# PositronicsLab/Moby

Measured on NVIDIA B200. Metric: env_steps_per_s, higher is better.
Workload: dtype f64

## Files before the change

include/b200moby.h:

```cpp
#ifndef B200MOBY_H
#define B200MOBY_H

#ifdef __cplusplus
extern "C" {
#endif

#define B200MOBY_ABI_VERSION 3

typedef enum {
  B200MOBY_OK = 0,
  B200MOBY_ERR_INVALID = 1,
  B200MOBY_ERR_CUDA = 2,
  B200MOBY_ERR_UNSUPPORTED = 3,
  B200MOBY_ERR_NO_DEVICE = 4
} b200moby_status;

enum {
  B200MOBY_LCP_OK = 0,
  B200MOBY_LCP_TRIVIAL = 1,
  B200MOBY_LCP_RAY = 2,
  B200MOBY_LCP_MAXITER = 3,
  B200MOBY_LCP_SINGULAR = 4,
  B200MOBY_LCP_EMPTY_RATIO = 5,
  B200MOBY_LCP_UNVERIFIED = 6,
// ... 100 lines not shown
b200moby_status b200moby_get_time(b200moby_handle h, double* t);
b200moby_status b200moby_get_last_lcp(b200moby_handle h, int* n, double* z, int zcap);

#define B200MOBY_MAX_KERNELS 20
typedef struct {
  char name[48];
  double ms;
  long long launches;
  long long envs;
  long long flops;
  long long lcp_solves;
  int lcp_nmax;
  int threads_per_env;
} b200moby_kernel_stat;
typedef struct {
  int n_kernels;
  b200moby_kernel_stat k[B200MOBY_MAX_KERNELS];
} b200moby_kernel_profile;
b200moby_status b200moby_get_kernel_profile(b200moby_handle h, int enable, int reset, b200moby_kernel_profile* out);

b200moby_status b200moby_get_impact_profile(b200moby_handle h, long long* prof);

b200moby_status b200moby_get_env_stats(b200moby_handle h, int* stat);

b200moby_status b200moby_lcp_lemke_batched(int batch, int n, const double* M_dev, const double* q_dev, double* z_dev,
                                           double piv_tol, double zero_tol, int* status_dev, int* pivots_dev,
                                           int* pivot_log_dev, int log_cap, void* stream);
b200moby_status b200moby_lcp_fast_batched(int batch, int n, const double* M_dev, const double* q_dev, double* z_dev,
                                          int warm_start, double zero_tol, int* status_dev, int* pivots_dev,
                                          int* pivot_log_dev, int log_cap, void* stream);
b200moby_status b200moby_lcp_lemke_regularized_batched(int batch, int n, const double* M_dev, const double* q_dev,
                                                       double* z_dev, int min_exp, int step_exp, int max_exp,
                                                       double piv_tol, double zero_tol, int* status_dev,
                                                       int* pivots_dev, void* stream);
b200moby_status b200moby_lcp_fast_regularized_batched(int batch, int n, const double* M_dev, const double* q_dev,
                                                      double* z_dev, int warm_start, int min_exp, int step_exp,
                                                      int max_exp, double zero_tol, int* status_dev, int* pivots_dev,
                                                      void* stream);
b200moby_status b200moby_lcp_lemke_host(int batch, int n, const double* M, const double* q, double* z, double piv_tol,
                                        double zero_tol, int* status, int* pivots, int device);
b200moby_status b200moby_lcp_fast_host(int batch, int n, const double* M, const double* q, double* z, int warm_start,
                                       double zero_tol, int* status, int* pivots, int device);

b200moby_status b200moby_selftest_div(int n, const double* x_dev, const double* y_dev, double* q_dev, double* qref_dev, void* stream);

b200moby_status b200moby_lcp_solve_host(int mode, int batch, int n, const double* M, const double* q, double* z, int warm_start,
// ... 20 lines not shown
```

moby_b200/capi.py:

```python
import ctypes as C
import os

_HERE = os.path.dirname(os.path.abspath(__file__))
LIB_PATH = os.environ.get("B200MOBY_LIB", os.path.join(_HERE, "libb200moby.so"))


class B200MobyError(RuntimeError):
    pass


class RcDesc(C.Structure):
    _fields_ = [
        ("n_links", C.c_int), ("first_body", C.c_int),
        ("parent", C.POINTER(C.c_int)), ("joint_type", C.POINTER(C.c_int)),
        ("joint_axis", C.POINTER(C.c_double)), ("loc_parent", C.POINTER(C.c_double)), ("loc_child", C.POINTER(C.c_double)),
        ("rel_quat", C.POINTER(C.c_double)),
        ("fdyn_algorithm", C.c_int),
        ("ctrl_kp", C.POINTER(C.c_double)), ("ctrl_kv", C.POINTER(C.c_double)), ("ctrl_amp", C.POINTER(C.c_double)),
        ("ctrl_freq", C.POINTER(C.c_double)),
    ]


class SceneDesc(C.Structure):
    _fields_ = [
# ... 14 lines not shown
    _fields_ = [("name", C.c_char * 48), ("ms", C.c_double), ("launches", C.c_longlong), ("envs", C.c_longlong),
                ("flops", C.c_longlong), ("lcp_solves", C.c_longlong), ("lcp_nmax", C.c_int), ("threads_per_env", C.c_int)]


class KernelProfile(C.Structure):
    _fields_ = [("n_kernels", C.c_int), ("k", KernelStat * 20)]


class Counters(C.Structure):
    _fields_ = [(k, C.c_longlong) for k in (
        "env_steps", "mini_steps", "lcp_solves", "lcp_fast_calls", "lemke_calls", "pivots", "lcp_failures",
        "impact_tol_events", "contacts", "max_lcp_n", "pivot_flops", "ca_iterations", "assembly_flops", "stab_iterations",
        "stab_lcp_solves", "stab_line_search_failures")]

    def as_dict(self):
        return {k: int(getattr(self, k)) for k, _ in self._fields_}


SYMBOLS = [
    "b200moby_last_error", "b200moby_abi_version", "b200moby_device_count",
    "b200moby_create", "b200moby_destroy", "b200moby_set_state", "b200moby_get_state",
    "b200moby_set_state_dev", "b200moby_get_state_dev", "b200moby_step", "b200moby_set_pivot_budget", "b200moby_get_counters",
    "b200moby_reset_counters", "b200moby_get_launch_count", "b200moby_get_time", "b200moby_get_last_lcp",
    "b200moby_get_impact_profile", "b200moby_get_kernel_profile", "b200moby_get_env_stats",
    "b200moby_lcp_lemke_batched", "b200moby_lcp_fast_batched", "b200moby_lcp_lemke_regularized_batched",
    "b200moby_lcp_fast_regularized_batched", "b200moby_lcp_lemke_host", "b200moby_lcp_fast_host", "b200moby_lcp_solve_host",
    "b200moby_selftest_div",
    "b200moby_fwd_dyn_batched", "b200moby_find_contacts_batched", "b200moby_find_contacts_host", "b200moby_delassus_batched",
    "b200moby_set_joint_state", "b200moby_get_joint_state", "b200moby_set_joint_state_dev", "b200moby_get_joint_state_dev",
    "b200moby_set_joint_forces", "b200moby_rc_fwd_dyn_batched", "b200moby_rc_inertia_batched",
]

_lib = None


def lib():
    global _lib
    if _lib is not None:
        return _lib
    if not os.path.exists(LIB_PATH):
        raise B200MobyError(f"{LIB_PATH} not built; run `python -c 'import __graft_entry__ as g; g.build()'` "
                            "(there is no CPU fallback for the hot path)")
    L = C.CDLL(LIB_PATH)
    L.b200moby_last_error.restype = C.c_char_p
    vp, ip, dp = C.c_void_p, C.c_void_p, C.c_void_p
    L.b200moby_create.argtypes = [C.POINTER(SceneDesc), C.c_int, C.POINTER(C.c_void_p)]
    L.b200moby_destroy.argtypes = [C.c_void_p]
    L.b200moby_set_state.argtypes = [C.c_void_p, dp, dp]
    L.b200moby_get_state.argtypes = [C.c_void_p, dp, dp]
    L.b200moby_set_state_dev.argtypes = [C.c_void_p, dp, dp, vp]
    L.b200moby_get_state_dev.argtypes = [C.c_void_p, dp, dp, vp]
    L.b200moby_step.argtypes = [C.c_void_p, C.c_double, C.c_int, vp]
    L.b200moby_set_pivot_budget.argtypes = [C.c_void_p, C.c_int]
    L.b200moby_get_counters.argtypes = [C.c_void_p, C.POINTER(Counters)]
    L.b200moby_reset_counters.argtypes = [C.c_void_p]
    L.b200moby_get_launch_count.argtypes = [C.c_void_p, C.POINTER(C.c_longlong)]
    L.b200moby_get_time.argtypes = [C.c_void_p, dp]
    L.b200moby_get_last_lcp.argtypes = [C.c_void_p, ip, dp, C.c_int]
    L.b200moby_get_impact_profile.argtypes = [C.c_void_p, ip]
    L.b200moby_get_env_stats.argtypes = [C.c_void_p, ip]
    L.b200moby_get_kernel_profile.argtypes = [C.c_void_p, C.c_int, C.c_int, C.POINTER(KernelProfile)]
    L.b200moby_lcp_lemke_batched.argtypes = [C.c_int, C.c_int, dp, dp, dp, C.c_double, C.c_double, ip, ip, ip, C.c_int, vp]
    L.b200moby_lcp_fast_batched.argtypes = [C.c_int, C.c_int, dp, dp, dp, C.c_int, C.c_double, ip, ip, ip, C.c_int, vp]
    L.b200moby_lcp_lemke_regularized_batched.argtypes = [C.c_int, C.c_int, dp, dp, dp, C.c_int, C.c_int, C.c_int,
                                                         C.c_double, C.c_double, ip, ip, vp]
    L.b200moby_lcp_fast_regularized_batched.argtypes = [C.c_int, C.c_int, dp, dp, dp, C.c_int, C.c_int, C.c_int, C.c_int,
                                                        C.c_double, ip, ip, vp]
    L.b200moby_lcp_lemke_host.argtypes = [C.c_int, C.c_int, dp, dp, dp, C.c_double, C.c_double, ip, ip, C.c_int]
    L.b200moby_lcp_fast_host.argtypes = [C.c_int, C.c_int, dp, dp, dp, C.c_int, C.c_double, ip, ip, C.c_int]
    L.b200moby_lcp_solve_host.argtypes = [C.c_int, C.c_int, C.c_int, dp, dp, dp, C.c_int, C.c_double, C.c_double, C.c_int, C.c_int,
                                          C.c_int, ip, ip, C.c_int]
    L.b200moby_selftest_div.argtypes = [C.c_int, dp, dp, dp, dp, vp]
    L.b200moby_fwd_dyn_batched.argtypes = [C.c_void_p, dp, dp, C.c_double, vp]
    L.b200moby_find_contacts_batched.argtypes = [C.c_void_p, dp, dp, C.c_int, ip, dp, dp, dp, dp, ip, dp, vp]
    L.b200moby_find_contacts_host.argtypes = [C.c_void_p, C.c_int, ip, dp, dp, dp, dp, ip, dp]
    L.b200moby_delassus_batched.argtypes = [C.c_void_p, dp, dp, C.c_int, dp, dp, ip, vp]
    L.b200moby_set_joint_state.argtypes = [C.c_void_p, dp, dp]
    L.b200moby_get_joint_state.argtypes = [C.c_void_p, dp, dp]
    L.b200moby_set_joint_state_dev.argtypes = [C.c_void_p, dp, dp, vp]
    L.b200moby_get_joint_state_dev.argtypes = [C.c_void_p, dp, dp, vp]
    L.b200moby_set_joint_forces.argtypes = [C.c_void_p, dp]
    L.b200moby_rc_fwd_dyn_batched.argtypes = [C.c_void_p, C.c_int, dp, dp, dp, dp, vp]
    L.b200moby_rc_inertia_batched.argtypes = [C.c_void_p, dp, dp, vp]
# ... 8 lines not shown
```

moby_b200/csrc/lcp_device.cuh:

```cuda
#pragma once
#include "common.cuh"

namespace b2m {

enum {
  LCP_OK = 0, LCP_TRIVIAL = 1, LCP_RAY = 2, LCP_MAXITER = 3, LCP_SINGULAR = 4, LCP_EMPTY_RATIO = 5,
  LCP_UNVERIFIED = 6, LCP_DEFER = 7, LCP_REGULARIZED = 16
};

B2M_DEV B2M_INL double m_at(const double* M, int ldm, int r, int c, double lambda) {
  double v = M[(size_t)c * ldm + r];
  return (r == c) ? v + lambda : v;
}

template <class G>
B2M_DEV B2M_NOINL double norm_inf(const G& g, int n, const double* M, int ldm, double lambda) {
  double m = 0.0;
  if constexpr (G::size == 1) {
    double m1 = 0.0, m2 = 0.0, m3 = 0.0;
    for (int c = 0; c < n; c++) {
      const double* Mc = M + (size_t)c * ldm;
      int r = 0;
      for (; r + 8 <= n; r += 8) {
        double v0 = Mc[r], v1 = Mc[r + 1], v2 = Mc[r + 2], v3 = Mc[r + 3], v4 = Mc[r + 4], v5 = Mc[r + 5], v6 = Mc[r + 6], v7 = Mc[r + 7];
// ... 664 lines not shown
    }
#endif
    for (int i = j + 1 + g.tid; i < k; i += G::size) {
      const double l = A[(size_t)j * k + i] * rinv;
      A[(size_t)j * k + i] = l;
      for (int c = j + 1; c < k; c++) A[(size_t)c * k + i] = fma(-l, A[(size_t)c * k + j], A[(size_t)c * k + i]);
      b[i] = fma(-l, bj, b[i]);
    }
    g.sync();
  }
  for (int c = k - 1; c >= 0; c--) {
    const double xc = b[c] / A[(size_t)c * k + c];
    g.sync();
    if (g.tid == 0) b[c] = xc;
    for (int i = g.tid; i < c; i += G::size) b[i] = fma(-A[(size_t)c * k + i], xc, b[i]);
    g.sync();
  }
  return true;
}

B2M_DEV inline void list_erase(int* L, int& m, int pos) { for (int i = pos; i + 1 < m; i++) L[i] = L[i + 1]; m--; }
B2M_DEV inline void list_insert_sorted(int* L, int& m, int v) { int i = m; while (i > 0 && L[i - 1] > v) { L[i] = L[i - 1]; i--; } L[i] = v; m++; }

template <class G>
B2M_DEV B2M_NOINL int lcp_fast_solve(const G& g, int n, const double* M, int ldm, const double* q, double lambda, double zero_tol,
                              bool warm, double* z, double* wd, int* wi, int* pivots_out, int* log, int log_cap,
                              int* log_len, int* budget = nullptr, int* executed_out = nullptr, double offdiag = -1.0) {
  double* A = wd;
  double* zz = A + (size_t)n * n;
  double* w = zz + n;
  int* nonbas = wi;
  int* bas = wi + n;
  int* cnt = wi + 2 * n;
  const int W32 = (n + 31) >> 5;
  unsigned* cur = (unsigned*)(wi + 2 * n + 2);
  unsigned* hist = cur + W32;
  int nlog = 0, nh = 0, executed = 0;
  if (executed_out) *executed_out = 0;
  if (zero_tol < 0.0) zero_tol = n * norm_inf_with(g, n, M, ldm, lambda, offdiag) * B2M_EPS;
  if (warm) {
    if (g.tid == 0) {
      int k = 0, nb = 0;
      for (int i = 0; i < W32; i++) cur[i] = 0u;
      for (int i = 0; i < n; i++) { if (fabs(z[i]) < zero_tol) bas[nb++] = i; else { nonbas[k++] = i; cur[i >> 5] |= 1u << (i & 31); } }
      cnt[0] = k; cnt[1] = nb;
    }
  } else {
    double key = B2M_INF; int idx = 0x7fffffff;
    for (int i = g.tid; i < n; i += G::size) { const double x = q[i]; if (x < key) { key = x; idx = i; } }
    g.min_key_idx(key, idx);
    if (key > -zero_tol) {
      for (int i = g.tid; i < n; i += G::size) z[i] = 0.0;
      if (pivots_out) *pivots_out = 0; if (log_len) *log_len = 0;
      g.sync();
      return LCP_TRIVIAL;
    }
    if (g.tid == 0) {
      nonbas[0] = idx; int nb = 0; for (int i = 0; i < n; i++) if (i != idx) bas[nb++] = i; cnt[0] = 1; cnt[1] = nb;
      for (int i = 0; i < W32; i++) cur[i] = 0u;
      cur[idx >> 5] |= 1u << (idx & 31);
    }
  }
  g.sync();
  const int MAX_PIV = 2 * n;
  int piv = 0, status = LCP_MAXITER;
  for (piv = 0; piv < MAX_PIV; piv++) {
    if (budget && --(*budget) < 0) { status = LCP_DEFER; break; }
    {
      bool rep = false;
      if (!log) {
        const int stored = nh < B2M_FAST_HIST ? nh : B2M_FAST_HIST;
        for (int t = g.tid; t < stored; t += G::size) {
          bool eq = true;
          for (int i = 0; i < W32; i++) eq = eq && (hist[t * W32 + i] == cur[i]);
          rep = rep || eq;
        }
      }
      if (g.any(rep)) { piv = MAX_PIV; break; }
      if (!log) { for (int i = g.tid; i < W32; i += G::size) hist[(nh % B2M_FAST_HIST) * W32 + i] = cur[i]; nh++; }
    }
    executed++;
    const int k = cnt[0], nb = cnt[1];
    if (G::size == 32 && k <= 64) {
      const double* __restrict__ Mr = M; const int* __restrict__ nbp = nonbas; double* __restrict__ Ar = A;
      for (int r = g.tid; r < k; r += G::size) {
        const int nr = nbp[r];
#pragma unroll 4
        for (int c = 0; c < k; c++) Ar[c * k + r] = m_at(Mr, ldm, nr, nbp[c], lambda);
      }
    } else if (G::size == 1) {
// ... 171 lines not shown
    case 9: return 1e9;
    case 10: return 1e10;
    case 11: return 1e11;
    case 12: return 1e12;
    case 13: return 1e13;
    case 14: return 1e14;
    case 15: return 1e15;
    case 16: return 1e16;
    case 17: return 1e17;
    case 18: return 1e18;
    case 19: return 1e19;
    case 20: return 1e20;
    case 21: return 1e21;
    case 22: return 1e22;
    case 23: return 1e23;
    case 24: return 1e24;
    default: return pow(10.0, (double)e);
  }
}

template <class G>
B2M_DEV int lcp_fast_regularized(const G& g, int n, const double* M, int ldm, const double* q, double zero_tol, bool warm,
                                    int min_exp, int step_exp, int max_exp, double* z, double* wd, int* wi,
                                    int* pivots_out, long long* stats, int* budget = nullptr) {
  if (n == 0) { if (pivots_out) *pivots_out = 0; return LCP_OK; }
  const double offdiag = norm_inf_offdiag(g, n, M, ldm);
  const double ZERO_TOL = (zero_tol > 0.0) ? zero_tol : n * norm_inf_with(g, n, M, ldm, 0.0, offdiag) * B2M_NEAR_ZERO;
  double* wv = wd + (size_t)n * n + n;
  int total = 0, piv = 0, ex = 0;
  int st = lcp_fast_solve(g, n, M, ldm, q, 0.0, zero_tol, warm, z, wd, wi, &piv, nullptr, 0, nullptr, budget, &ex, offdiag);
  if (st == LCP_DEFER) return st;
  bool zvalid = warm || st == LCP_OK || st == LCP_TRIVIAL;
  total += piv;
  if (stats && g.tid == 0) { stats[0]++; stats[1] += piv; stats[2] += ex; }
  if ((st == LCP_OK || st == LCP_TRIVIAL) && lcp_verify(g, n, M, ldm, q, 0.0, z, ZERO_TOL, false, wv)) {
    if (pivots_out) *pivots_out = piv;
    return st;
  }
  int attempt = 0;
  for (int rf = min_exp; rf < max_exp; rf += step_exp, attempt++) {
    const double lambda = pow10i(rf);
    g.sync();
    st = lcp_fast_solve(g, n, M, ldm, q, lambda, zero_tol, zvalid, z, wd, wi, &piv, nullptr, 0, nullptr, budget, &ex, offdiag);
    if (st == LCP_DEFER) return st;
    zvalid = zvalid || st == LCP_OK || st == LCP_TRIVIAL;
    total += piv;
    if (stats && g.tid == 0) { stats[0]++; stats[1] += piv; stats[2] += ex; }
    if ((st == LCP_OK || st == LCP_TRIVIAL) && lcp_verify(g, n, M, ldm, q, lambda, z, ZERO_TOL, true, wv)) {
      if (pivots_out) *pivots_out = total;
      return LCP_REGULARIZED + attempt;
    }
  }
  if (pivots_out) *pivots_out = total;
  return LCP_UNVERIFIED;
}

template <class G>
B2M_DEV int lcp_lemke_regularized(const G& g, int n, const double* M, int ldm, const double* q, double piv_tol,
                                     double zero_tol, int min_exp, int step_exp, int max_exp, double* z, double* wd,
                                     int* wi, int* pivots_out, long long* stats, int* budget = nullptr) {
  if (n == 0) { if (pivots_out) *pivots_out = 0; return LCP_OK; }
  const double offdiag = norm_inf_offdiag(g, n, M, ldm);
  const double ZERO_TOL = (zero_tol > 0.0) ? zero_tol : n * norm_inf_with(g, n, M, ldm, 0.0, offdiag) * B2M_NEAR_ZERO;
  double* wv = wd + (size_t)n * (n + 2);
  int total = 0, piv = 0, ex = 0;
  int st = lemke_solve(g, n, M, ldm, q, 0.0, piv_tol, zero_tol, z, wd, wi, &piv, nullptr, 0, nullptr, budget, &ex, offdiag);
  if (st == LCP_DEFER) return st;
// ... 210 lines not shown
```

moby_b200/csrc/sim_device.cuh:

```cuda
#pragma once
#include "lcp_device.cuh"
#include "rc_device.cuh"

namespace b2m {

enum { SH_NONE = 0, SH_SPHERE = 1, SH_BOX = 2, SH_PLANE = 3,
       SH_WHEEL = 4,
       SH_PIN = 5, SH_PINWORLD = 6 };
enum { CNT_ENV_STEPS = 0, CNT_MINI_STEPS, CNT_LCP_SOLVES, CNT_FAST_CALLS, CNT_LEMKE_CALLS, CNT_PIVOTS, CNT_LCP_FAIL,
       CNT_IMPACT_TOL, CNT_CONTACTS, CNT_MAX_N, CNT_OVERFLOW, CNT_PIVOT_FLOPS, CNT_ASM_FLOPS, CNT_CA_ITERS, CNT_STAB_ITERS, CNT_STAB_SOLVES, CNT_STAB_LSFAIL, CNT_COUNT };
#define B2M_NKMAX 64
#define B2M_WHEEL_NS_MAX 16
#define B2M_WTAB_OFF ((size_t)4 * (B2M_NKMAX + 1) * (B2M_NKMAX / 2))
#define B2M_MAX_CLASSES 12
#define B2M_SLOT_CONT B2M_MAX_CLASSES
#define B2M_SLOT_STRAGGLER (B2M_MAX_CLASSES + 1)
#define B2M_SLOT_HARD (B2M_MAX_CLASSES + 2)
#define B2M_SLOT_HARD_BACK (B2M_MAX_CLASSES + 3)
#define B2M_SLOTS (B2M_MAX_CLASSES + 4)
#define B2M_ROUNDS_MAX 8
#define B2M_MAX_STALL 64
#ifndef B2M_LEAN
#define B2M_LEAN 0
#endif
// ... 28 lines not shown
  int stab_max_iterations; double stab_eps;
  const double* min_step_env;
  double* q; double* v; double* time; double* zlast; int* zlast_n;
  double* vlast; int* vlast_n;
  unsigned long long* counters;
  int* cost; int hard_cost; int cost_shift;
  int thread_lanes;
  int pivot_budget;
  double* hacc;
  double* hpend;
  int* queue;
  int* qctl;
  int n_classes; int class_nmax[B2M_MAX_CLASSES]; int class_cmax[B2M_MAX_CLASSES];
  int class_budget[B2M_MAX_CLASSES];
  double* tap_MM; double* tap_qq; double* tap_z; int* tap_n;
  const RCTree* rc; int rc_links, rc_first;
  int ngc;
  double* jq; double* jqd; const double* jtau;
  double* gscratch; size_t gstride;
  unsigned long long* kstat; int kslot;
  int* env_stat;
  int tap_times;
  long long* tap_prof;
};

struct EnvMem {
  double *bx, *bq, *bR, *bvl, *bva, *bmass, *bdims, *bJ, *xsave, *qsave;
  double *pd_dist, *pd_pa, *pd_pb;
  double *cp, *cnrm, *ct1, *ct2, *cdist, *cmu, *cmuv, *ceps, *ccomp;
  double *Jr, *XJ, *Xb, *D, *Cv, *imp, *acc, *dv;
  double *MM, *qq, *z, *zl, *vl, *work;
  double *Lf, *gv;
  double *jq, *jqd, *jqsave, *jtau, *rS, *rV;
  int *bshape, *ben, *pair_a, *pair_b, *cb1, *cb2, *cNK, *icon, *cisl, *corder, *isl_start, *gcoff, *bisl, *frow_c, *frow_j, *scal, *iwork;
  int *ranc, *gcb, *gcl;
  long long* prof; long long prof_stride;
  const double* wtab;
  long long dbg[4];
  double cdt;
};

enum { PH_LOAD = 0, PH_CONTACTS, PH_ISLANDS, PH_PROBLEM, PH_BUILD, PH_FAST, PH_LEMKE, PH_APPLY, PH_STORE, PH_COUNT };
#ifdef __CUDA_ARCH__
#define B2M_PROF_T0(m) const long long _pt0 = (m).prof ? clock64() : 0
#define B2M_PROF_ADD(m, g, k) do { if ((m).prof && (g).tid == 0) (m).prof[(k) * (m).prof_stride] += clock64() - _pt0; } while (0)
#else
// ... 38 lines not shown
  m.Jr = nullptr; m.zl = nullptr; m.vl = nullptr; m.prof = nullptr; m.prof_stride = 0; m.gcb = m.gcl = nullptr; m.cdt = 0.0; m.wtab = nullptr;
}
B2M_HD inline void env_carve_impact(EnvMem& m, double* d, int* i, const EnvDims& D) {
  const int nb = D.nb, cmax = D.cmax, nmax = D.nmax;
  if (D.ngc) { m.Jr = d; d += (size_t)3 * cmax * D.ngc; m.XJ = d; d += (size_t)3 * cmax * D.ngc; m.Xb = d; d += (size_t)D.ngc * D.ngc; m.dv = d; d += D.ngc; m.Lf = d; d += (size_t)D.ngc * D.ngc + D.ngc; m.gv = d; d += D.ngc; }
  else { m.Lf = m.gv = nullptr; m.Jr = d; d += 36 * cmax; m.XJ = d; d += 36 * cmax; m.Xb = d; d += 36 * nb; m.dv = d; d += 6 * nb; }
  m.D = d; d += 6 * (size_t)cmax * cmax;
  m.Cv = d; d += 3 * cmax; m.imp = d; d += 3 * cmax; m.acc = d; d += 3 * cmax;
  m.MM = d; d += (size_t)nmax * nmax; m.qq = d; d += nmax; m.z = d; d += nmax; m.zl = d; d += nmax; m.vl = d; d += cmax; m.work = d;
  m.gcoff = i; i += nb; m.bisl = i; i += nb;
  m.icon = i; i += cmax; m.cisl = i; i += cmax; m.corder = i; i += cmax;
  m.isl_start = i; i += nb + 1;
  m.frow_c = i; i += nmax; m.frow_j = i; i += nmax;
  m.gcb = i; i += D.ngc; m.gcl = i; i += D.ngc;
  m.iwork = i;
}
B2M_HD inline void env_carve(EnvMem& m, double* d, int* i, const EnvDims& D) {
  env_carve_small(m, d, i, D);
  env_carve_impact(m, d + env_small_doubles(D), i + env_small_ints(D), D);
}

enum { S_NPAIRS = 0, S_NCON = 1, S_NC = 2, S_NGC = 3, S_N = 4, S_NISL = 5, S_FLAG = 6, S_TMP = 7, S_ZLN = 8, S_ZLDIRTY = 9, S_NTOT = 10, S_VLN = 11, S_VLDIRTY = 12, S_FAILED = 13, S_EXEC = 14 };

struct EnvCtx { int budget; bool limit; void* ladder = nullptr; };

struct EnvStatBase { unsigned long long fail, lemke, fast, solves, pivots; };
B2M_HD B2M_INL EnvStatBase env_stat_base(const unsigned long long* lc);

B2M_HD B2M_INL EnvStatBase env_stat_base(const unsigned long long* lc) {
  EnvStatBase b; b.fail = lc[CNT_LCP_FAIL] + lc[CNT_OVERFLOW]; b.lemke = lc[CNT_LEMKE_CALLS]; b.fast = lc[CNT_FAST_CALLS]; b.solves = lc[CNT_LCP_SOLVES]; b.pivots = lc[CNT_PIVOTS]; return b;
}
template <class G>
B2M_DEV B2M_INL void env_stat_commit(const G& g, const SimParams& P, int e, const unsigned long long* lc, const EnvStatBase& b) {
  if (!P.env_stat || g.tid != 0) return;
  const size_t ne = P.n_envs;
  P.env_stat[e] += (int)(lc[CNT_LCP_FAIL] + lc[CNT_OVERFLOW] - b.fail);
  P.env_stat[ne + e] += (int)(lc[CNT_LEMKE_CALLS] - b.lemke);
  P.env_stat[2 * ne + e] += (int)(lc[CNT_FAST_CALLS] - b.fast);
  P.env_stat[3 * ne + e] += (int)(lc[CNT_LCP_SOLVES] - b.solves);
  P.env_stat[4 * ne + e] += (int)(lc[CNT_PIVOTS] - b.pivots);
}

B2M_HD B2M_INL void quat_to_R(const double* qt, double* R) {
  const double x = qt[0], y = qt[1], z = qt[2], w = qt[3];
  R[0] = 1.0 - 2.0 * (y * y + z * z); R[1] = 2.0 * (x * y - w * z);       R[2] = 2.0 * (x * z + w * y);
  R[3] = 2.0 * (x * y + w * z);       R[4] = 1.0 - 2.0 * (x * x + z * z); R[5] = 2.0 * (y * z - w * x);
  R[6] = 2.0 * (x * z - w * y);       R[7] = 2.0 * (y * z + w * x);       R[8] = 1.0 - 2.0 * (x * x + y * y);
// ... 1146 lines not shown
}

template <class G>
B2M_DEV double min_constraint_velocity(const G& g, const EnvMem& m) {
  const int nc = m.scal[S_NC];
  double v = B2M_INF;
  for (int i = g.tid; i < nc; i += G::size) v = fmin(v, m.Cv[i]);
  return g.min(v);
}

template <class G>
B2M_DEV B2M_NOINL bool solve_qp(const G& g, const SimParams& P, int e, EnvMem& m, unsigned long long* lc, EnvCtx& cx) {
  const int nc = m.scal[S_NC];
  int n;
  { B2M_PROF_T0(m); n = build_qp_lcp(g, P, m); B2M_PROF_ADD(m, g, PH_BUILD); }
  if (n > P.nmax) { if (g.tid == 0) { lc[CNT_OVERFLOW]++; } for (int t = g.tid; t < 3 * nc; t += G::size) m.imp[t] = 0.0; g.sync(); return true; }
  const bool warm = (m.scal[S_ZLN] == n);
  for (int i = g.tid; i < n; i += G::size) m.z[i] = warm ? m.zl[i] : 0.0;
  g.sync();
  long long stats[3] = {0, 0, 0};
  int piv = 0;
  int* bud = cx.limit ? &cx.budget : nullptr;
  int st;
#ifdef __CUDA_ARCH__
#define B2M_STAMP(row) do { if (m.prof && P.tap_times && g.tid == 0) { long long _gt; asm volatile("mov.u64 %0, %%globaltimer;" : "=l"(_gt)); m.prof[(row) * m.prof_stride] = _gt; } } while (0)
#else
#define B2M_STAMP(row) do {} while (0)
#endif
  B2M_STAMP(PH_CONTACTS);
  { B2M_PROF_T0(m); st = lcp_fast_regularized(g, n, m.MM, n, m.qq, -1.0, true, -20, 4, -8, m.z, m.work, m.iwork, &piv, stats, bud); B2M_PROF_ADD(m, g, PH_FAST); }
  B2M_STAMP(PH_PROBLEM);
  if (st == LCP_DEFER) return false;
  long long fast_calls = stats[0], pivots = stats[1], executed = stats[2], lemke_calls = 0;
  if (st == LCP_UNVERIFIED) {
    g.sync();
    stats[0] = stats[1] = stats[2] = 0;
    { B2M_PROF_T0(m);
#ifdef __CUDACC__
      if constexpr (G::size >= 32) {
        if (cx.ladder) {
          LadderCtx LC = *(const LadderCtx*)cx.ladder;
          if (m.prof && P.tap_times) LC.dbg = m.dbg;
          st = lcp_lemke_regularized_pool(g, LC, n, m.MM, n, m.qq, -1.0, -1.0, -20, 1, 1, m.z, &piv, stats);
        }
        else st = lcp_lemke_regularized(g, n, m.MM, n, m.qq, -1.0, -1.0, -20, 1, 1, m.z, m.work, m.iwork, &piv, stats, bud);
      } else
#endif
      st = lcp_lemke_regularized(g, n, m.MM, n, m.qq, -1.0, -1.0, -20, 1, 1, m.z, m.work, m.iwork, &piv, stats, bud);
      B2M_PROF_ADD(m, g, PH_LEMKE); }
    if (st == LCP_DEFER) return false;
    B2M_STAMP(PH_BUILD);
    lemke_calls = stats[0]; pivots += stats[1]; executed += stats[2];
    if (st == LCP_UNVERIFIED) { for (int i = g.tid; i < n; i += G::size) m.z[i] = 0.0; if (g.tid == 0) { lc[CNT_LCP_FAIL]++; m.scal[S_FAILED] = 1; } }
  }
  g.sync();
  if (g.tid == 0) {
    lc[CNT_LCP_SOLVES]++; lc[CNT_FAST_CALLS] += fast_calls; lc[CNT_LEMKE_CALLS] += lemke_calls; lc[CNT_PIVOTS] += pivots;
    lc[CNT_PIVOT_FLOPS] += (unsigned long long)executed * 2ull * n * (n + 1);
    m.scal[S_EXEC] += (int)executed;
    if ((unsigned long long)n > lc[CNT_MAX_N]) lc[CNT_MAX_N] = n;
    m.scal[S_ZLN] = n; m.scal[S_ZLDIRTY] = 1;
  }
  for (int i = g.tid; i < n; i += G::size) m.zl[i] = m.z[i];
  if (P.tap_n) {
    if (g.tid == 0) P.tap_n[e] = n;
    for (int t = g.tid; t < n * n; t += G::size) P.tap_MM[(size_t)e * P.nmax * P.nmax + t] = m.MM[t];
    for (int i = g.tid; i < n; i += G::size) { P.tap_qq[(size_t)e * P.nmax + i] = m.qq[i]; P.tap_z[(size_t)e * P.nmax + i] = m.z[i]; }
  }
  for (int i = g.tid; i < nc; i += G::size) {
    m.imp[i] = m.z[i];
    m.imp[nc + i] = m.z[nc + i] - m.z[3 * nc + i];
    m.imp[2 * nc + i] = m.z[2 * nc + i] - m.z[4 * nc + i];
  }
// ... 449 lines not shown
  if (g.tid == 0) P.time[e] = t;
  g.sync();
}

template <class G>
B2M_DEV bool env_impact(const G& g, const SimParams& P, int e, EnvMem& m, double dt, int round, unsigned long long* lc, EnvCtx& cx) {
#ifdef __CUDA_ARCH__
  const long long t0 = P.tap_prof ? clock64() : 0;
  long long gt0 = 0;
  if (P.tap_prof && P.tap_times) asm volatile("mov.u64 %0, %%globaltimer;" : "=l"(gt0));
#endif
  const unsigned long long p0 = lc[CNT_PIVOTS], f0 = lc[CNT_PIVOT_FLOPS];
  const EnvStatBase sb = env_stat_base(lc);
  m.prof = P.tap_prof ? P.tap_prof + (size_t)4 * P.n_envs + e : nullptr; m.prof_stride = P.n_envs;
  { B2M_PROF_T0(m); env_load(g, P, e, m); B2M_PROF_ADD(m, g, PH_LOAD); }
  const unsigned long long c0 = lc[CNT_CONTACTS], o0 = lc[CNT_OVERFLOW];
  if (g.tid == 0) { m.scal[S_FAILED] = 0; m.scal[S_EXEC] = 0; }
  m.dbg[0] = m.dbg[1] = m.dbg[2] = m.dbg[3] = 0;
  { B2M_PROF_T0(m);
  calc_pairwise_distances(g, m);
  find_unilateral_constraints(g, P, e, m, lc);
  B2M_PROF_ADD(m, g, PH_CONTACTS); }
  lc[CNT_CONTACTS] = c0; lc[CNT_OVERFLOW] = o0;
  if (!process_constraints(g, P, e, m, lc, cx)) {
    if (g.tid == 0) { const int hc = P.pivot_budget > P.hard_cost ? P.pivot_budget : P.hard_cost; q_push(P, round, B2M_SLOT_STRAGGLER, e); if (P.cost && P.cost[e] < 4 * hc) P.cost[e] = 4 * hc; }
    g.sync();
    return false;
  }
  mini_step_account(g, P, m, lc);
  env_stat_commit(g, P, e, lc, sb);
  g.sync();
  { B2M_PROF_T0(m); env_store(g, P, e, m, ST_VEL | ST_ZL); B2M_PROF_ADD(m, g, PH_STORE); }
  if (g.tid == 0) {
    const double hh = P.hpend[e];
    const double h = P.hacc[e] + hh;
    P.time[e] = P.time[e] + hh;
    if (h < dt && !(hh == 0.0 && m.scal[S_FAILED])) { P.hacc[e] = h; q_push(P, round, B2M_SLOT_CONT, e); }
    else lc[CNT_ENV_STEPS]++;
    if (P.cost) { const int prev = P.cost[e], dec = prev - (prev >> P.cost_shift); P.cost[e] = m.scal[S_EXEC] > dec ? m.scal[S_EXEC] : dec; }
#ifdef __CUDA_ARCH__
    if (P.tap_prof) {
      const size_t ne = P.n_envs;
      const long long n = m.scal[S_N];
      P.tap_prof[e] = clock64() - t0; P.tap_prof[ne + e] = (long long)(lc[CNT_PIVOTS] - p0);
      P.tap_prof[2 * ne + e] = n > 0 ? (long long)((lc[CNT_PIVOT_FLOPS] - f0) / (2ull * n * (n + 1))) : 0; P.tap_prof[3 * ne + e] = n + 1000ll * P.kslot;
      if (P.tap_times) {
        long long gt1; asm volatile("mov.u64 %0, %%globaltimer;" : "=l"(gt1));
        P.tap_prof[(4 + PH_ISLANDS) * ne + e] = gt0; P.tap_prof[(4 + PH_STORE) * ne + e] = gt1;
        P.tap_prof[(4 + PH_APPLY) * ne + e] = m.dbg[0]; P.tap_prof[(4 + PH_LOAD) * ne + e] = m.dbg[1]; P.tap_prof[(4 + PH_LEMKE) * ne + e] = m.dbg[2] + 1000 * m.dbg[3];
      }
    }
// ... 24 lines not shown
```

moby_b200/csrc/sim_kernels.cu:

```cuda
#include <atomic>
#include <cstdio>
#include <cstdlib>
#include <cstring>
#include <vector>
#include <nvtx3/nvToolsExt.h>
#include "friction_table.h"
#include "host_util.h"
#include "sim_kernel_util.cuh"
#include "rc_host.h"

using namespace b2m;

#define B2M_SMEM_MAX (227 * 1024 - 1024)

struct ClassPlan {
  int nmax = 0, cmax = 0;
  int threads = 32;
  int tvariant = -1;
  int wpb = 1, grid = 1;
  size_t shmem = 0;
  double* gscratch = nullptr;
  size_t gstride = 0;
};

// ... 508 lines not shown
  TRY(dev_copy(h, tab.data(), tab.size(), &P.fr_tab));
  P.gx = d->gravity[0]; P.gy = d->gravity[1]; P.gz = d->gravity[2];
  P.contact_dist_thresh = d->contact_dist_thresh; P.min_step_size = d->min_step_size;
  P.stab_max_iterations = d->stabilization_max_iterations; P.stab_eps = B2M_NEAR_ZERO;
  if (d->min_step_size_env) TRY(dev_copy(h, d->min_step_size_env, (size_t)ne, &P.min_step_env));
  TRY(dev_zero(h, (size_t)nb * 7 * ne, &P.q));
  TRY(dev_zero(h, (size_t)nb * 6 * ne, &P.v));
  TRY(dev_zero(h, (size_t)ne, &P.time));
  TRY(dev_zero(h, (size_t)h->nmax * ne, &P.zlast));
  TRY(dev_zero(h, (size_t)ne, &P.zlast_n));
  TRY(dev_zero(h, (size_t)h->cmax * ne, &P.vlast));
  TRY(dev_zero(h, (size_t)ne, &P.vlast_n));
  TRY(dev_zero(h, (size_t)CNT_COUNT, &P.counters));
  TRY(dev_zero(h, (size_t)3 * (B2M_MAX_CLASSES + 6), &P.kstat));
  TRY(dev_zero(h, (size_t)ne, &P.cost));
  P.tap_times = env_int("B200MOBY_TAP_TIMES", 0);
  P.hard_cost = env_int("B200MOBY_HARD_COST", 12);
  P.cost_shift = std::max(0, std::min(30, env_int("B200MOBY_COST_DECAY_SHIFT", 2)));
  TRY(dev_zero(h, (size_t)ne, &P.hacc));
  TRY(dev_zero(h, (size_t)ne, &P.hpend));
  TRY(dev_zero(h, (size_t)B2M_ROUNDS_MAX * B2M_SLOTS * ne, &P.queue));
  TRY(dev_zero(h, (size_t)2 * B2M_ROUNDS_MAX * (B2M_SLOTS + 1), &P.qctl));
  P.pivot_budget = env_int("B200MOBY_PIVOT_BUDGET", 96);
  if (d->rc && d->rc->n_links > 0) {
    const b200moby_rc_desc& r = *d->rc;
    RCTree T; bool unsup = false;
    if (const char* err = b2m_rc_tree_from_desc(r, nb, T, &unsup)) { b200moby_destroy(h); return b2m_fail(unsup ? B200MOBY_ERR_UNSUPPORTED : B200MOBY_ERR_INVALID, "%s", err); }
    for (int e = 0; e < ne; e++) {
      if (d->enabled[(size_t)r.first_body * ne + e]) { b200moby_destroy(h); return b2m_fail(B200MOBY_ERR_UNSUPPORTED, "articulated body: floating bases are not on the accelerated path; the base link must be a disabled body"); }
      for (int i = 1; i < r.n_links; i++) if (!d->enabled[(size_t)(r.first_body + i) * ne + e]) { b200moby_destroy(h); return b2m_fail(B200MOBY_ERR_INVALID, "articulated body: link %d is disabled", i); }
    }
    TRY(dev_copy(h, &T, 1, &P.rc));
    P.rc_links = r.n_links; P.rc_first = r.first_body;
    P.ngc = b2m_dense_ngc(d);
    h->rc_links = r.n_links; h->rc_dof = r.n_links - 1;
    TRY(dev_zero(h, (size_t)h->rc_dof * ne, &P.jq));
    TRY(dev_zero(h, (size_t)h->rc_dof * ne, &P.jqd));
    double* tau0 = nullptr;
    TRY(dev_zero(h, (size_t)h->rc_dof * ne, &tau0));
    P.jtau = tau0;
  }
  TRY(plan_launch(h));
  h->concurrent = env_int("B200MOBY_CONCURRENT", 1) != 0;
  h->graph_on = env_int("B200MOBY_GRAPH", h->rounds <= 2 ? 1 : 0) != 0;
  if (h->concurrent) {
    h->side.resize(h->classes.size()); h->side_done.resize(h->classes.size());
// ... 185 lines not shown
}

b200moby_status b200moby_get_counters(b200moby_handle h, b200moby_counters* out) {
  if (!h || !out) return b2m_fail(B200MOBY_ERR_INVALID, "null argument");
  unsigned long long c[CNT_COUNT];
  B2M_CUDA(cudaSetDevice(h->device));
  B2M_CUDA(cudaMemcpy(c, h->P.counters, sizeof(c), cudaMemcpyDeviceToHost));
  out->env_steps = c[CNT_ENV_STEPS]; out->mini_steps = c[CNT_MINI_STEPS]; out->lcp_solves = c[CNT_LCP_SOLVES];
  out->lcp_fast_calls = c[CNT_FAST_CALLS]; out->lemke_calls = c[CNT_LEMKE_CALLS]; out->pivots = c[CNT_PIVOTS];
  out->lcp_failures = c[CNT_LCP_FAIL] + c[CNT_OVERFLOW]; out->impact_tol_events = c[CNT_IMPACT_TOL]; out->contacts = c[CNT_CONTACTS];
  out->max_lcp_n = c[CNT_MAX_N]; out->pivot_flops = c[CNT_PIVOT_FLOPS]; out->assembly_flops = c[CNT_ASM_FLOPS]; out->ca_iterations = c[CNT_CA_ITERS];
  out->stab_iterations = c[CNT_STAB_ITERS]; out->stab_lcp_solves = c[CNT_STAB_SOLVES]; out->stab_line_search_failures = c[CNT_STAB_LSFAIL];
  return B200MOBY_OK;
}
b200moby_status b200moby_get_launch_count(b200moby_handle h, long long* out) {
  if (!h || !out) return b2m_fail(B200MOBY_ERR_INVALID, "null argument");
  *out = h->launches;
  return B200MOBY_OK;
}
b200moby_status b200moby_reset_counters(b200moby_handle h) {
  if (!h) return b2m_fail(B200MOBY_ERR_INVALID, "null handle");
  B2M_CUDA(cudaSetDevice(h->device));
  B2M_CUDA(cudaMemset(h->P.counters, 0, sizeof(unsigned long long) * CNT_COUNT));
  return B200MOBY_OK;
}
b200moby_status b200moby_get_time(b200moby_handle h, double* t) {
  if (!h || !t) return b2m_fail(B200MOBY_ERR_INVALID, "null argument");
  B2M_CUDA(cudaSetDevice(h->device));
  B2M_CUDA(cudaMemcpy(t, h->P.time, sizeof(double) * h->n_envs, cudaMemcpyDeviceToHost));
  return B200MOBY_OK;
}

b200moby_status b200moby_get_last_lcp(b200moby_handle h, int* n, double* z, int zcap) {
  if (!h) return b2m_fail(B200MOBY_ERR_INVALID, "null handle");
  B2M_CUDA(cudaSetDevice(h->device));
  if (!h->taps) {
    b200moby_status st;
    if ((st = dev_zero(h, (size_t)h->n_envs * h->nmax * h->nmax, &h->P.tap_MM)) != B200MOBY_OK) return st;
    if ((st = dev_zero(h, (size_t)h->n_envs * h->nmax, &h->P.tap_qq)) != B200MOBY_OK) return st;
    if ((st = dev_zero(h, (size_t)h->n_envs * h->nmax, &h->P.tap_z)) != B200MOBY_OK) return st;
    if ((st = dev_zero(h, (size_t)h->n_envs, &h->P.tap_n)) != B200MOBY_OK) return st;
    h->taps = true;
  }
  if (n) B2M_CUDA(cudaMemcpy(n, h->P.tap_n, sizeof(int) * h->n_envs, cudaMemcpyDeviceToHost));
  if (z) {
    std::vector<double> tmp((size_t)h->n_envs * h->nmax);
// ... 116 lines not shown
```

moby_b200/simulator.py:

```python
import ctypes as C

import numpy as np

from . import capi


class TimeSteppingSimulator:
    def __init__(self, scene, device=0):
        self.scene = scene
        self.device = device
        self.contact_dist_thresh = scene.contact_dist_thresh
        self.min_step_size = scene.min_step_size
        self.post_step_callback_fn = None
        self._desc = scene.cdesc()
        self._h = C.c_void_p()
        capi.check(capi.lib().b200moby_create(C.byref(self._desc), device, C.byref(self._h)))
        self.n_envs, self.n_bodies = scene.n_envs, scene.n_bodies
        self.set_state(scene.q, scene.v)
        self.rc = getattr(scene, "rc", None)
        if self.rc is not None:
            self.set_joint_state(self.rc.jq, self.rc.jqd)
        self.steps_taken = 0

    def close(self):
# ... 89 lines not shown
        capi.check(capi.lib().b200moby_get_launch_count(self._h, C.byref(n)))
        return int(n.value)

    def reset_counters(self):
        capi.check(capi.lib().b200moby_reset_counters(self._h))

    def kernel_profile(self, enable=True, reset=True):
        kp = capi.KernelProfile()
        capi.check(capi.lib().b200moby_get_kernel_profile(self._h, int(enable), int(reset), C.byref(kp)))
        return [dict(name=kp.k[i].name.decode(), ms=kp.k[i].ms, launches=kp.k[i].launches, envs=kp.k[i].envs, flops=kp.k[i].flops,
                     lcp_solves=kp.k[i].lcp_solves, lcp_nmax=kp.k[i].lcp_nmax, threads_per_env=kp.k[i].threads_per_env)
                for i in range(kp.n_kernels)]

    def impact_profile(self):
        prof = np.zeros((13, self.n_envs), np.int64)
        capi.check(capi.lib().b200moby_get_impact_profile(self._h, prof.ctypes.data))
        return prof

    def env_stats(self):
        st = np.zeros((5, self.n_envs), np.int32)
        capi.check(capi.lib().b200moby_get_env_stats(self._h, st.ctypes.data))
        return dict(lcp_failures=st[0], lemke_calls=st[1], lcp_fast_calls=st[2], lcp_solves=st[3], pivots=st[4])

    def last_lcp_z(self, zcap):
        n = np.zeros(self.n_envs, np.int32)
        z = np.zeros((self.n_envs, zcap))
        capi.check(capi.lib().b200moby_get_last_lcp(self._h, n.ctypes.data, z.ctypes.data, zcap))
        return n, z

    def fwd_dyn(self, q, v, dt, stream=None):
        capi.check(capi.lib().b200moby_fwd_dyn_batched(self._h, q.data_ptr(), v.data_ptr(), float(dt), _stream(stream)))

    def find_contacts(self, q, v, cap, stream=None):
        import torch
        ne, dev = self.n_envs, q.device
        count = torch.zeros(ne, dtype=torch.int32, device=dev)
        pt, nr, t1, t2 = (torch.zeros((cap, 3, ne), dtype=torch.float64, device=dev) for _ in range(4))
        pair = torch.zeros((cap, ne), dtype=torch.int32, device=dev)
        dist = torch.zeros((cap, ne), dtype=torch.float64, device=dev)
        capi.check(capi.lib().b200moby_find_contacts_batched(self._h, q.data_ptr(), v.data_ptr(), cap, count.data_ptr(), pt.data_ptr(),
                                                             nr.data_ptr(), t1.data_ptr(), t2.data_ptr(), pair.data_ptr(),
                                                             dist.data_ptr(), _stream(stream)))
        return dict(count=count, point=pt, normal=nr, tan1=t1, tan2=t2, pair=pair, dist=dist)

    def delassus(self, q, v, nmax, stream=None):
        import torch
# ... 20 lines not shown
```

Baseline: 7.609 million.

## Checkpoint deferred fast-LCP pivot state so straggler reruns resume instead of restarting

When the budgeted fast LCP solver runs out of pivot budget, the solver state (basis lists, pivot history, z, rung, counters) is saved per environment in global memory. The straggler pass then resumes from that state instead of re-running the pivots it already did, and for Lemke-phase defers it skips the fast phase. This avoids repeating pivot work for deferred environments, at the cost of extra global writes and reads on defer, extra per-env memory, and atomic counters for resume statistics.

After: 7.638 million, median of 6. Within noise of the previous version (+0.4%).

```diff
diff --git a/include/b200moby.h b/include/b200moby.h
--- a/include/b200moby.h
+++ b/include/b200moby.h
@@ -146,6 +146,7 @@
 b200moby_status b200moby_get_impact_profile(b200moby_handle h, long long* prof);
 
 b200moby_status b200moby_get_env_stats(b200moby_handle h, int* stat);
+b200moby_status b200moby_get_resume_stats(b200moby_handle h, unsigned long long* out);
 
 b200moby_status b200moby_lcp_lemke_batched(int batch, int n, const double* M_dev, const double* q_dev, double* z_dev,
                                            double piv_tol, double zero_tol, int* status_dev, int* pivots_dev,
diff --git a/moby_b200/capi.py b/moby_b200/capi.py
--- a/moby_b200/capi.py
+++ b/moby_b200/capi.py
@@ -60,7 +60,7 @@
     "b200moby_create", "b200moby_destroy", "b200moby_set_state", "b200moby_get_state",
     "b200moby_set_state_dev", "b200moby_get_state_dev", "b200moby_step", "b200moby_set_pivot_budget", "b200moby_get_counters",
     "b200moby_reset_counters", "b200moby_get_launch_count", "b200moby_get_time", "b200moby_get_last_lcp",
-    "b200moby_get_impact_profile", "b200moby_get_kernel_profile", "b200moby_get_env_stats",
+    "b200moby_get_impact_profile", "b200moby_get_kernel_profile", "b200moby_get_env_stats", "b200moby_get_resume_stats",
     "b200moby_lcp_lemke_batched", "b200moby_lcp_fast_batched", "b200moby_lcp_lemke_regularized_batched",
     "b200moby_lcp_fast_regularized_batched", "b200moby_lcp_lemke_host", "b200moby_lcp_fast_host", "b200moby_lcp_solve_host",
     "b200moby_selftest_div",
@@ -97,6 +97,7 @@
     L.b200moby_get_last_lcp.argtypes = [C.c_void_p, ip, dp, C.c_int]
     L.b200moby_get_impact_profile.argtypes = [C.c_void_p, ip]
     L.b200moby_get_env_stats.argtypes = [C.c_void_p, ip]
+    L.b200moby_get_resume_stats.argtypes = [C.c_void_p, vp]
     L.b200moby_get_kernel_profile.argtypes = [C.c_void_p, C.c_int, C.c_int, C.POINTER(KernelProfile)]
     L.b200moby_lcp_lemke_batched.argtypes = [C.c_int, C.c_int, dp, dp, dp, C.c_double, C.c_double, ip, ip, ip, C.c_int, vp]
     L.b200moby_lcp_fast_batched.argtypes = [C.c_int, C.c_int, dp, dp, dp, C.c_int, C.c_double, ip, ip, ip, C.c_int, vp]
diff --git a/moby_b200/csrc/lcp_device.cuh b/moby_b200/csrc/lcp_device.cuh
--- a/moby_b200/csrc/lcp_device.cuh
+++ b/moby_b200/csrc/lcp_device.cuh
@@ -710,10 +710,18 @@
 B2M_DEV inline void list_erase(int* L, int& m, int pos) { for (int i = pos; i + 1 < m; i++) L[i] = L[i + 1]; m--; }
 B2M_DEV inline void list_insert_sorted(int* L, int& m, int v) { int i = m; while (i > 0 && L[i - 1] > v) { L[i] = L[i - 1]; i--; } L[i] = v; m++; }
 
+struct FastResume {
+  int rung;
+  int zvalid, total;
+  int piv, executed, nh;
+  bool resume;
+};
+
 template <class G>
 B2M_DEV B2M_NOINL int lcp_fast_solve(const G& g, int n, const double* M, int ldm, const double* q, double lambda, double zero_tol,
                               bool warm, double* z, double* wd, int* wi, int* pivots_out, int* log, int log_cap,
-                              int* log_len, int* budget = nullptr, int* executed_out = nullptr, double offdiag = -1.0) {
+                              int* log_len, int* budget = nullptr, int* executed_out = nullptr, double offdiag = -1.0,
+                              FastResume* rs = nullptr) {
   double* A = wd;
   double* zz = A + (size_t)n * n;
   double* w = zz + n;
@@ -726,7 +734,14 @@
   int nlog = 0, nh = 0, executed = 0;
   if (executed_out) *executed_out = 0;
   if (zero_tol < 0.0) zero_tol = n * norm_inf_with(g, n, M, ldm, lambda, offdiag) * B2M_EPS;
-  if (warm) {
+  const bool resume = rs && rs->resume;
+  if (resume) {
+    nh = rs->nh; executed = rs->executed;
+    if (g.tid == 0) {
+      for (int i = 0; i < W32; i++) cur[i] = 0u;
+      for (int i = 0; i < cnt[0]; i++) cur[nonbas[i] >> 5] |= 1u << (nonbas[i] & 31);
+    }
+  } else if (warm) {
     if (g.tid == 0) {
       int k = 0, nb = 0;
       for (int i = 0; i < W32; i++) cur[i] = 0u;
@@ -751,9 +766,13 @@
   }
   g.sync();
   const int MAX_PIV = 2 * n;
-  int piv = 0, status = LCP_MAXITER;
-  for (piv = 0; piv < MAX_PIV; piv++) {
-    if (budget && --(*budget) < 0) { status = LCP_DEFER; break; }
+  int piv = resume ? rs->piv : 0, status = LCP_MAXITER;
+  for (; piv < MAX_PIV; piv++) {
+    if (budget && --(*budget) < 0) {
+      status = LCP_DEFER;
+      if (rs) { rs->piv = piv; rs->executed = executed; rs->nh = nh; }
+      break;
+    }
     {
       bool rep = false;
       if (!log) {
@@ -971,27 +990,35 @@
 template <class G>
 B2M_DEV int lcp_fast_regularized(const G& g, int n, const double* M, int ldm, const double* q, double zero_tol, bool warm,
                                     int min_exp, int step_exp, int max_exp, double* z, double* wd, int* wi,
-                                    int* pivots_out, long long* stats, int* budget = nullptr) {
+                                    int* pivots_out, long long* stats, int* budget = nullptr, FastResume* rs = nullptr) {
   if (n == 0) { if (pivots_out) *pivots_out = 0; return LCP_OK; }
   const double offdiag = norm_inf_offdiag(g, n, M, ldm);
   const double ZERO_TOL = (zero_tol > 0.0) ? zero_tol : n * norm_inf_with(g, n, M, ldm, 0.0, offdiag) * B2M_NEAR_ZERO;
   double* wv = wd + (size_t)n * n + n;
   int total = 0, piv = 0, ex = 0;
-  int st = lcp_fast_solve(g, n, M, ldm, q, 0.0, zero_tol, warm, z, wd, wi, &piv, nullptr, 0, nullptr, budget, &ex, offdiag);
-  if (st == LCP_DEFER) return st;
-  bool zvalid = warm || st == LCP_OK || st == LCP_TRIVIAL;
-  total += piv;
-  if (stats && g.tid == 0) { stats[0]++; stats[1] += piv; stats[2] += ex; }
-  if ((st == LCP_OK || st == LCP_TRIVIAL) && lcp_verify(g, n, M, ldm, q, 0.0, z, ZERO_TOL, false, wv)) {
-    if (pivots_out) *pivots_out = piv;
-    return st;
-  }
+  const int first = (rs && rs->resume) ? rs->rung : 0;
+  bool zvalid = warm;
+  int st;
+  if (first == 0) {
+    st = lcp_fast_solve(g, n, M, ldm, q, 0.0, zero_tol, warm, z, wd, wi, &piv, nullptr, 0, nullptr, budget, &ex, offdiag, rs);
+    if (st == LCP_DEFER) { if (rs) { rs->rung = 0; rs->zvalid = zvalid; rs->total = total; } return st; }
+    if (rs) rs->resume = false;
+    zvalid = warm || st == LCP_OK || st == LCP_TRIVIAL;
+    total += piv;
+    if (stats && g.tid == 0) { stats[0]++; stats[1] += piv; stats[2] += ex; }
+    if ((st == LCP_OK || st == LCP_TRIVIAL) && lcp_verify(g, n, M, ldm, q, 0.0, z, ZERO_TOL, false, wv)) {
+      if (pivots_out) *pivots_out = piv;
+      return st;
+    }
+  } else { zvalid = rs->zvalid != 0; total = rs->total; }
   int attempt = 0;
   for (int rf = min_exp; rf < max_exp; rf += step_exp, attempt++) {
+    if (1 + attempt < first) continue;
     const double lambda = pow10i(rf);
     g.sync();
-    st = lcp_fast_solve(g, n, M, ldm, q, lambda, zero_tol, zvalid, z, wd, wi, &piv, nullptr, 0, nullptr, budget, &ex, offdiag);
-    if (st == LCP_DEFER) return st;
+    st = lcp_fast_solve(g, n, M, ldm, q, lambda, zero_tol, zvalid, z, wd, wi, &piv, nullptr, 0, nullptr, budget, &ex, offdiag, rs);
+    if (st == LCP_DEFER) { if (rs) { rs->rung = 1 + attempt; rs->zvalid = zvalid; rs->total = total; } return st; }
+    if (rs) rs->resume = false;
     zvalid = zvalid || st == LCP_OK || st == LCP_TRIVIAL;
     total += piv;
     if (stats && g.tid == 0) { stats[0]++; stats[1] += piv; stats[2] += ex; }
diff --git a/moby_b200/csrc/sim_device.cuh b/moby_b200/csrc/sim_device.cuh
--- a/moby_b200/csrc/sim_device.cuh
+++ b/moby_b200/csrc/sim_device.cuh
@@ -74,6 +74,8 @@
   int* env_stat;
   int tap_times;
   long long* tap_prof;
+  int* rs_i; double* rs_z; int rs_nmax;
+  unsigned long long* rs_stat;
 };
 
 struct EnvMem {
@@ -158,7 +160,20 @@
 
 enum { S_NPAIRS = 0, S_NCON = 1, S_NC = 2, S_NGC = 3, S_N = 4, S_NISL = 5, S_FLAG = 6, S_TMP = 7, S_ZLN = 8, S_ZLDIRTY = 9, S_NTOT = 10, S_VLN = 11, S_VLDIRTY = 12, S_FAILED = 13, S_EXEC = 14 };
 
-struct EnvCtx { int budget; bool limit; void* ladder = nullptr; };
+struct EnvCtx { int budget; bool limit; void* ladder = nullptr; int solve_ord = 0; int resume_ord = 0; };
+
+enum { RS_ORD = 0, RS_PHASE, RS_RUNG, RS_ZVALID, RS_TOTAL, RS_ST0, RS_ST1, RS_ST2, RS_PIV, RS_EXEC, RS_NH, RS_K, RS_NB, RS_LISTS };
+B2M_HD inline int fast_hist_words(int n) { return B2M_FAST_HIST * ((n + 31) >> 5); }
+B2M_HD inline size_t resume_rec_ints(int nmax) { return (size_t)RS_LISTS + 2 * (size_t)nmax + fast_hist_words(nmax); }
+enum { RS_STAT_DEFER = 0, RS_STAT_DEFER_ITERS, RS_STAT_WRITTEN, RS_STAT_RESUME_FAST, RS_STAT_RESUME_LEMKE, RS_STAT_SKIPPED, RS_STAT_COUNT };
+B2M_DEV B2M_INL void rs_stat_add(const SimParams& P, int k, unsigned long long v) {
+  if (!P.rs_stat) return;
+#ifdef __CUDA_ARCH__
+  atomicAdd(P.rs_stat + k, v);
+#else
+  P.rs_stat[k] += v;
+#endif
+}
 
 struct EnvStatBase { unsigned long long fail, lemke, fast, solves, pivots; };
 B2M_HD B2M_INL EnvStatBase env_stat_base(const unsigned long long* lc);
@@ -1351,15 +1366,54 @@
   int piv = 0;
   int* bud = cx.limit ? &cx.budget : nullptr;
   int st;
+  const int ord = ++cx.solve_ord;
+  const size_t ne = P.n_envs;
+  FastResume rs; rs.resume = false;
+  const bool record = cx.limit && P.rs_i;
+  int phase = 0;
+  if (cx.resume_ord == ord) {
+    const int* R = P.rs_i + e;
+    phase = R[RS_PHASE * ne];
+    stats[0] = R[RS_ST0 * ne]; stats[1] = R[RS_ST1 * ne]; stats[2] = R[RS_ST2 * ne];
+    if (phase == 0) {
+      rs.resume = true; rs.rung = R[RS_RUNG * ne]; rs.zvalid = R[RS_ZVALID * ne]; rs.total = R[RS_TOTAL * ne];
+      rs.piv = R[RS_PIV * ne]; rs.executed = R[RS_EXEC * ne]; rs.nh = R[RS_NH * ne];
+      const int W = fast_hist_words(n), W32 = (n + 31) >> 5;
+      for (int i = g.tid; i < 2 * n; i += G::size) m.iwork[i] = R[(RS_LISTS + i) * ne];
+      for (int i = g.tid; i < W; i += G::size) m.iwork[2 * n + 2 + W32 + i] = R[(RS_LISTS + 2 * P.rs_nmax + i) * ne];
+      if (g.tid == 0) { m.iwork[2 * n] = R[RS_K * ne]; m.iwork[2 * n + 1] = R[RS_NB * ne]; }
+      for (int i = g.tid; i < n; i += G::size) m.z[i] = P.rs_z[i * ne + e];
+      if (g.tid == 0) { rs_stat_add(P, RS_STAT_RESUME_FAST, 1); rs_stat_add(P, RS_STAT_SKIPPED, (unsigned long long)(stats[2] + rs.executed)); }
+    } else if (g.tid == 0) { rs_stat_add(P, RS_STAT_RESUME_LEMKE, 1); rs_stat_add(P, RS_STAT_SKIPPED, (unsigned long long)stats[2]); }
+    g.sync();
+  }
 #ifdef __CUDA_ARCH__
 #define B2M_STAMP(row) do { if (m.prof && P.tap_times && g.tid == 0) { long long _gt; asm volatile("mov.u64 %0, %%globaltimer;" : "=l"(_gt)); m.prof[(row) * m.prof_stride] = _gt; } } while (0)
 #else
 #define B2M_STAMP(row) do {} while (0)
 #endif
   B2M_STAMP(PH_CONTACTS);
-  { B2M_PROF_T0(m); st = lcp_fast_regularized(g, n, m.MM, n, m.qq, -1.0, true, -20, 4, -8, m.z, m.work, m.iwork, &piv, stats, bud); B2M_PROF_ADD(m, g, PH_FAST); }
+  if (phase == 0) {
+    B2M_PROF_T0(m); st = lcp_fast_regularized(g, n, m.MM, n, m.qq, -1.0, true, -20, 4, -8, m.z, m.work, m.iwork, &piv, stats, bud, (record || rs.resume) ? &rs : nullptr); B2M_PROF_ADD(m, g, PH_FAST);
+  } else st = LCP_UNVERIFIED;
   B2M_STAMP(PH_PROBLEM);
-  if (st == LCP_DEFER) return false;
+  if (st == LCP_DEFER) {
+    if (record) {
+      int* R = P.rs_i + e;
+      const int W = fast_hist_words(n), W32 = (n + 31) >> 5;
+      for (int i = g.tid; i < 2 * n; i += G::size) R[(RS_LISTS + i) * ne] = m.iwork[i];
+      for (int i = g.tid; i < W; i += G::size) R[(RS_LISTS + 2 * P.rs_nmax + i) * ne] = m.iwork[2 * n + 2 + W32 + i];
+      for (int i = g.tid; i < n; i += G::size) P.rs_z[i * ne + e] = m.z[i];
+      if (g.tid == 0) {
+        R[RS_ORD * ne] = ord; R[RS_PHASE * ne] = 0; R[RS_RUNG * ne] = rs.rung; R[RS_ZVALID * ne] = rs.zvalid; R[RS_TOTAL * ne] = rs.total;
+        R[RS_ST0 * ne] = (int)stats[0]; R[RS_ST1 * ne] = (int)stats[1]; R[RS_ST2 * ne] = (int)stats[2];
+        R[RS_PIV * ne] = rs.piv; R[RS_EXEC * ne] = rs.executed; R[RS_NH * ne] = rs.nh; R[RS_K * ne] = m.iwork[2 * n]; R[RS_NB * ne] = m.iwork[2 * n + 1];
+        rs_stat_add(P, RS_STAT_WRITTEN, 1);
+      }
+    }
+    g.sync();
+    return false;
+  }
   long long fast_calls = stats[0], pivots = stats[1], executed = stats[2], lemke_calls = 0;
   if (st == LCP_UNVERIFIED) {
     g.sync();
@@ -1377,7 +1431,16 @@
 #endif
       st = lcp_lemke_regularized(g, n, m.MM, n, m.qq, -1.0, -1.0, -20, 1, 1, m.z, m.work, m.iwork, &piv, stats, bud);
       B2M_PROF_ADD(m, g, PH_LEMKE); }
-    if (st == LCP_DEFER) return false;
+    if (st == LCP_DEFER) {
+      if (record && g.tid == 0) {
+        int* R = P.rs_i + e;
+        R[RS_ORD * ne] = ord; R[RS_PHASE * ne] = 1;
+        R[RS_ST0 * ne] = (int)fast_calls; R[RS_ST1 * ne] = (int)pivots; R[RS_ST2 * ne] = (int)executed;
+        rs_stat_add(P, RS_STAT_WRITTEN, 1);
+      }
+      g.sync();
+      return false;
+    }
     B2M_STAMP(PH_BUILD);
     lemke_calls = stats[0]; pivots += stats[1]; executed += stats[2];
     if (st == LCP_UNVERIFIED) { for (int i = g.tid; i < n; i += G::size) m.z[i] = 0.0; if (g.tid == 0) { lc[CNT_LCP_FAIL]++; m.scal[S_FAILED] = 1; } }
@@ -1873,11 +1936,17 @@
   find_unilateral_constraints(g, P, e, m, lc);
   B2M_PROF_ADD(m, g, PH_CONTACTS); }
   lc[CNT_CONTACTS] = c0; lc[CNT_OVERFLOW] = o0;
+  cx.solve_ord = 0;
+  cx.resume_ord = (!cx.limit && P.rs_i) ? P.rs_i[(size_t)RS_ORD * P.n_envs + e] : 0;
   if (!process_constraints(g, P, e, m, lc, cx)) {
-    if (g.tid == 0) { const int hc = P.pivot_budget > P.hard_cost ? P.pivot_budget : P.hard_cost; q_push(P, round, B2M_SLOT_STRAGGLER, e); if (P.cost && P.cost[e] < 4 * hc) P.cost[e] = 4 * hc; }
+    if (g.tid == 0) {
+      const int hc = P.pivot_budget > P.hard_cost ? P.pivot_budget : P.hard_cost; q_push(P, round, B2M_SLOT_STRAGGLER, e); if (P.cost && P.cost[e] < 4 * hc) P.cost[e] = 4 * hc;
+      rs_stat_add(P, RS_STAT_DEFER, 1); rs_stat_add(P, RS_STAT_DEFER_ITERS, (unsigned long long)P.pivot_budget);
+    }
     g.sync();
     return false;
   }
+  if (cx.resume_ord && g.tid == 0) P.rs_i[(size_t)RS_ORD * P.n_envs + e] = 0;
   mini_step_account(g, P, m, lc);
   env_stat_commit(g, P, e, lc, sb);
   g.sync();
diff --git a/moby_b200/csrc/sim_kernels.cu b/moby_b200/csrc/sim_kernels.cu
--- a/moby_b200/csrc/sim_kernels.cu
+++ b/moby_b200/csrc/sim_kernels.cu
@@ -554,6 +554,12 @@
   TRY(dev_zero(h, (size_t)B2M_ROUNDS_MAX * B2M_SLOTS * ne, &P.queue));
   TRY(dev_zero(h, (size_t)2 * B2M_ROUNDS_MAX * (B2M_SLOTS + 1), &P.qctl));
   P.pivot_budget = env_int("B200MOBY_PIVOT_BUDGET", 96);
+  TRY(dev_zero(h, (size_t)RS_STAT_COUNT, &P.rs_stat));
+  if (env_int("B200MOBY_RESUME", 1) != 0 && P.model != 1) {
+    P.rs_nmax = h->nmax;
+    TRY(dev_zero(h, resume_rec_ints(h->nmax) * ne, &P.rs_i));
+    TRY(dev_zero(h, (size_t)h->nmax * ne, &P.rs_z));
+  }
   if (d->rc && d->rc->n_links > 0) {
     const b200moby_rc_desc& r = *d->rc;
     RCTree T; bool unsup = false;
@@ -785,6 +791,13 @@
   if (!h) return b2m_fail(B200MOBY_ERR_INVALID, "null handle");
   B2M_CUDA(cudaSetDevice(h->device));
   B2M_CUDA(cudaMemset(h->P.counters, 0, sizeof(unsigned long long) * CNT_COUNT));
+  B2M_CUDA(cudaMemset(h->P.rs_stat, 0, sizeof(unsigned long long) * RS_STAT_COUNT));
+  return B200MOBY_OK;
+}
+b200moby_status b200moby_get_resume_stats(b200moby_handle h, unsigned long long* out) {
+  if (!h || !out) return b2m_fail(B200MOBY_ERR_INVALID, "null argument");
+  B2M_CUDA(cudaSetDevice(h->device));
+  B2M_CUDA(cudaMemcpy(out, h->P.rs_stat, sizeof(unsigned long long) * RS_STAT_COUNT, cudaMemcpyDeviceToHost));
   return B200MOBY_OK;
 }
 b200moby_status b200moby_get_time(b200moby_handle h, double* t) {
diff --git a/moby_b200/simulator.py b/moby_b200/simulator.py
--- a/moby_b200/simulator.py
+++ b/moby_b200/simulator.py
@@ -135,6 +135,12 @@
         capi.check(capi.lib().b200moby_get_env_stats(self._h, st.ctypes.data))
         return dict(lcp_failures=st[0], lemke_calls=st[1], lcp_fast_calls=st[2], lcp_solves=st[3], pivots=st[4])
 
+    def resume_stats(self):
+        st = np.zeros(6, np.uint64)
+        capi.check(capi.lib().b200moby_get_resume_stats(self._h, st.ctypes.data))
+        return dict(deferred=int(st[0]), deferred_iterations=int(st[1]), records=int(st[2]), resumed_fast=int(st[3]),
+                    resumed_lemke=int(st[4]), skipped_iterations=int(st[5]))
+
     def last_lcp_z(self, zcap):
         n = np.zeros(self.n_envs, np.int32)
         z = np.zeros((self.n_envs, zcap))
```
